# kocurvik/mdrp

Hardware: AMD Instinct MI355X
Metric: image-pairs/sec (2000 corrs, 10k RANSAC iters) (higher is better)
Workload: dtype f64

## Files before the change

### mdrp_amd/csrc/mdrp_capi.hip

```cpp
#include "../../include/mdrp.h"
#include "mdrp_kernels.h"
#include "mdrp_classic.h"
#ifdef MDRP_SPLIT_TU
#define MDRP_INST extern
#include "mdrp_instances.h"
namespace mdrp {
MDRP_INSTANCES_FINAL_64
MDRP_INSTANCES_FINAL_256
MDRP_INSTANCES_CLASSIC
}
#endif

#include <algorithm>
#include <cmath>
#include <cstdio>
#include <cstdlib>
#include <cstddef>
#include <cstring>
#include <functional>
#include <map>
#include <memory>
#include <mutex>
#include <string>
#include <vector>
// ... 342 lines not shown
    CamDev *d_cams1 = reinterpret_cast<CamDev *>(pd + sz.off_cam1), *d_cams2 = reinterpret_cast<CamDev *>(pd + sz.off_cam2);
    int32_t *d_table_n = reinterpret_cast<int32_t *>(pd + sz.off_tn), *d_table_of = reinterpret_cast<int32_t *>(pd + sz.off_tof),
            *d_nper = reinterpret_cast<int32_t *>(pd + sz.off_nper);
    Counters *cnt = h->counters.as<Counters>();
    const size_t groups_max = ((size_t)n_max + 15) / 16;
    const int trig_cap = chunk_cap;

    {
        unsigned char *ph = h->params_host;
        std::memcpy(ph, tab_state.data(), sizeof(uint64_t) * n_tables);
        const bool cams = kind == MDRP_CALIB || kind == MDRP_RELPOSE_5PT || kind == MDRP_SHARED_6PT;
        if (cams) { std::memcpy(ph + sz.off_cam1, cam1, sizeof(CamDev) * batch); std::memcpy(ph + sz.off_cam2, cam2 ? cam2 : cam1, sizeof(CamDev) * batch); }
        else std::memset(ph + sz.off_cam1, 0, 2 * sizeof(CamDev) * (size_t)batch);
        std::memcpy(ph + sz.off_tn, tab_n.data(), sizeof(int32_t) * n_tables);
        std::memcpy(ph + sz.off_tof, table_of.data(), sizeof(int32_t) * batch);
        std::memcpy(ph + sz.off_nper, n_host, sizeof(int32_t) * batch);
        HIPCHK(hipMemcpyAsync(pd, ph, sz.params, hipMemcpyHostToDevice, s));
    }
    HIPCHK(hipEventRecord(h->ev_tables, s));

    RunParams rp;
    std::memset(&rp, 0, sizeof rp);
    rp.kind = kind; rp.solver = solver_for(kind, est_shift); rp.est_shift = est_shift;
    rp.score_initial = ro->score_initial_model ? 1 : 0;
    rp.batch = batch; rp.n_max = n_max;
    rp.max_iterations = ro->max_iterations; rp.min_iterations = ro->min_iterations;
    rp.dyn_mult = ro->dyn_num_trials_mult; rp.log_prob_missing = std::log(1.0 - ro->success_prob);
    rp.weight_sampson = ro->monodepth_weight_sampson > 0.0f ? (double)ro->monodepth_weight_sampson : 0.0;
    rp.final_max_it = (int)std::min<uint64_t>(bo->max_iterations, 1u << 30); rp.final_loss = bo->loss_type;
    rp.grad_tol = bo->gradient_tol; rp.step_tol = bo->step_tol; rp.lambda0 = bo->initial_lambda;
    rp.lambda_min = bo->min_lambda; rp.lambda_max = bo->max_lambda;
    rp.chunk_len = chunk_cap; rp.chunk_off = 0; rp.slot_stride = chunk_cap * mps; rp.super_len = chunk_cap; rp.chunk_start = 0;
    rp.mps = mps; rp.sample_sz = ssz;

    auto launch_prep = [&](int p0, int pc, hipStream_t ps_) {
        const size_t o2 = (size_t)2 * p0 * n_max, o1 = (size_t)p0 * n_max;
        double *pts_p = h->pts.as<double>() + o1 * PT_STRIDE;
        uint4 *rfrag_p = h->rfrag.as<uint4>() + (size_t)p0 * groups_max * 64;
        if (classic)
            hipLaunchKernelGGL(kc_prep, dim3(pc), dim3(256), 0, ps_, rp, x1 + o2, x2 + o2, d_nper + p0, d_table_of + p0, d_cams1 + p0, d_cams2 + p0,
                               ro->max_epipolar_error, bo->loss_scale, pts_p, h->st.as<PairState>() + p0, rfrag_p);
        else
            hipLaunchKernelGGL(k_prep, dim3(pc), dim3(256), 0, ps_, rp, x1 + o2, x2 + o2, d1 + o1, d2 + o1, d_nper + p0, d_table_of + p0, d_cams1 + p0, d_cams2 + p0,
                               ro->max_epipolar_error, ro->max_reproj_error, bo->loss_scale, pts_p, h->dep.as<double>() + 2 * o1, h->st.as<PairState>() + p0, rfrag_p);
    };
    if (!host) {
        launch_prep(0, batch, s);
        HIPCHK(hipGetLastError());
    }
    rp.inl_stat = classic ? nullptr : &cnt->progress.wish_sum;

    const bool lo_overlap = env_int("MDRP_LO_OVERLAP", 1) != 0;
    const bool use_bound = env_int("MDRP_BOUND", 1) != 0;
    const int lo_threads = env_int("MDRP_LO_THREADS", (batch_call >= 128 && n_max < 4096) ? 64 : 256);
    const int final_threads = env_int("MDRP_FINAL_THREADS", batch_call >= 4096 ? 64 : 256);
    const int mask_index = lm_mask_index_on(n_max);
    const int clm_list_stride = lm_list_stride(n_max);
    const size_t clm_list_bytes = (size_t)2 * clm_list_stride * sizeof(uint16_t);
    const bool fuse_env = env_int("MDRP_FUSE_TAIL", ((kind == MDRP_CALIB && est_shift) || h->fuse_disabled) ? 0 : 1) != 0;
    bool final_done = false;
    auto launch_final = [&](const int32_t *ready, int32_t *fin_done, unsigned long long ticks, unsigned long long *timeouts) {
        if (classic)
            MDRP_CLASSIC_LM_DISPATCH(kc_final, final_threads, kind, dim3(batch), clm_list_bytes, s, rp, h->st.as<PairState>(), h->pts.as<double>(), mask_dev, results_dev,
                                     ready, fin_done, ticks, timeouts, clm_list_stride);
        else
            MDRP_FINAL_DISPATCH(final_threads, rp.final_loss, kind, est_shift, dim3(batch), (mask_index ? lm_final_list_bytes(n_max) : lm_list_bytes(n_max)), s, rp,
                                h->st.as<PairState>(), h->pts.as<double>(), h->dep.as<double>(), mask_dev, results_dev, lm_list_stride(n_max), mask_index,
                                h->lm_stats.as<unsigned long long>() + 2, ready, fin_done, ticks, timeouts);
    };
    const size_t tile_bytes = SCORE_TILE_BYTES;

    uint64_t it0 = 0;
    uint64_t max_needed = 0;
    while (true) {
        uint64_t lens[mdrp_handle::NC_MAX] = {0};
        int n_chunks = 1;
        if (it0 < certain) {
            const uint64_t span = std::min<uint64_t>(certain - it0, (uint64_t)chunk_cap);
            uint64_t used = 0;
            n_chunks = 0;
            if (it0 == 0)
                for (uint64_t l : lead) {
                    if (used + 2 * l > span) break;
                    lens[n_chunks++] = l; used += l;
                }
            lens[n_chunks++] = span - used;
        } else {
            lens[0] = std::min<uint64_t>(std::min<uint64_t>(std::max<uint64_t>(max_needed, 256), ro->max_iterations - it0), (uint64_t)chunk_cap);
        }
        uint64_t super_len = 0;
        for (int c = 0; c < n_chunks; ++c) super_len += lens[c];
        if (it0 == 0) h->first_chunk = (int64_t)lens[0];
        rp.chunk_start = it0; rp.super_len = (int)super_len;
        HIPCHK(hipMemsetAsync(h->counters.p, 0, sizeof(Counters), s));
        if (it0 == 0) HIPCHK(hipMemsetAsync(h->cand_stat.p, 0, sizeof(unsigned long long) * 2 * batch, s));
        const bool piped = n_chunks > 1 && lo_overlap;
        const bool fuse_tail = fuse_env && piped && it0 + super_len >= ro->max_iterations;
        int32_t *fz_ctl = nullptr, *fz_done = nullptr, *fz_fin = nullptr, *fz_ready = nullptr;
        if (fuse_tail) {
            if ((rc = h->fuse.ensure(sz.fuse))) return rc;
            fz_ctl = h->fuse.as<int32_t>(); fz_done = fz_ctl + 16; fz_fin = fz_done + batch; fz_ready = fz_fin + batch;
        }
        hipStream_t aux = piped ? h->aux_stream : s, aux2 = piped ? h->aux_stream2 : s;
        int offs[mdrp_handle::NC_MAX] = {0};
        for (int c = 1; c < n_chunks; ++c) offs[c] = offs[c - 1] + (int)lens[c - 1];
        const int samp_threads = env_int("MDRP_SAMPLE_THREADS", ssz == 3 ? SAMP_THREADS : (ssz == 5 ? 512 : 256));
// ... 75 lines not shown
            int32_t *surv1 = h->surv_count.as<int32_t>() + p0, *surv2 = h->surv2_count.as<int32_t>() + p0;
            hipEvent_t e0, e1;
            int rc_;
            if ((rc_ = get_events(h, &e0, &e1, 0))) return rc_;
            unsigned long long *cstats = &cnt->progress.evals;
            {
                hipEvent_t c0, c1;
                if ((rc_ = get_events(h, &c0, &c1, 1))) return rc_;
                const bool two_phase = !(it0 == 0 && c == 0);
                unsigned long long *cand_stat = h->cand_stat.as<unsigned long long>() + 2 * (size_t)p0;
                uint32_t *tags_u = tags_sc;
                int32_t *und_part = reinterpret_cast<int32_t *>(h->tags_sorted[!odd].as<uint32_t>() + so), *und_cnt = h->und_count.as<int32_t>() + 2 * (size_t)p0;
                const uint4 *rfrag_p = h->rfrag.as<uint4>() + (size_t)p0 * groups_max * 64;
                hipLaunchKernelGGL(k_count_plan, dim3(1), dim3(PLAN_THREADS), 0, s, pc, st_p, mcount_c, 2, CNT_WG_MODELS, h->cplan.as<int32_t>(),
                                   surv1, (const int32_t *)nullptr, two_phase ? und_cnt : (int32_t *)nullptr);
                const dim3 cgrid((unsigned)pc * (unsigned)((len * mps + CNT_WG_MODELS - 1) / CNT_WG_MODELS));
                HIPCHK(hipEventRecord(c0, s));
                MDRP_SWEEP_DISPATCH(k_count, kind, cgrid, dim3(CNT_THREADS), 0, s, r, st_p, rfrag_p, models_p,
                                    tags_c, mcount_c, h->cplan.as<int32_t>(), tags_v, surv1, cstats, (int32_t *)nullptr, (const int32_t *)nullptr,
                                    1, tags_u, und_part, und_cnt, (const int32_t *)nullptr, cand_stat);
                if (two_phase) {
                    hipLaunchKernelGGL(k_count_plan, dim3(1), dim3(PLAN_THREADS), 0, s, pc, st_p, und_cnt, 2, CNT_WG_MODELS, h->cplan.as<int32_t>(),
                                       (int32_t *)nullptr, (const int32_t *)nullptr, (int32_t *)nullptr);
                    MDRP_SWEEP_DISPATCH(k_count, kind, cgrid, dim3(CNT_THREADS), 0, s, r, st_p, rfrag_p, models_p,
                                        tags_u, und_cnt, h->cplan.as<int32_t>(), tags_v, surv1, cstats, (int32_t *)nullptr, (const int32_t *)nullptr,
                                        2, (uint32_t *)nullptr, (int32_t *)nullptr, (int32_t *)nullptr, und_part, cand_stat);
                    h->count_launches++;
                }
                HIPCHK(hipEventRecord(c1, s));
                h->count_launches++;
            }
            const uint32_t *surv_tags = tags_v;
            const int32_t *surv_cnt = surv1;
            if (use_bound && batch_call > 16 && !(it0 == 0 && c == 0)) {
                hipLaunchKernelGGL(k_count_plan, dim3(1), dim3(PLAN_THREADS), 0, s, pc, st_p, surv1, 1, BND_THREADS, h->cplan.as<int32_t>(), surv2, (const int32_t *)nullptr);
                const dim3 bgrid((unsigned)pc * (unsigned)((len * mps + BND_THREADS - 1) / BND_THREADS));
                unsigned long long *bstats = &cnt->progress.evals_bound;
                hipEvent_t b0, b1;
                if ((rc_ = get_events(h, &b0, &b1, 4))) return rc_;
                HIPCHK(hipEventRecord(b0, s));
                MDRP_SWEEP_DISPATCH(k_bound, kind, bgrid, dim3(BND_THREADS), 0, s, r, st_p, pts_p, models_p, tags_v, surv1, h->cplan.as<int32_t>(), tags_c, surv2, bstats);
                HIPCHK(hipEventRecord(b1, s));
                surv_tags = tags_c; surv_cnt = surv2;
            }
            int32_t *plan = h->plan.as<int32_t>(), *totals = plan + 2 * (size_t)batch + 2;
            if (batch_call <= SCORE_WAVE_MAX_PAIRS) {
                hipLaunchKernelGGL(k_count_plan, dim3(1), dim3(PLAN_THREADS), 0, s, pc, st_p, surv_cnt, 1, SCW_THREADS / 64, plan, (int32_t *)nullptr, (const int32_t *)nullptr, (int32_t *)nullptr);
                hipLaunchKernelGGL(k_sort_tags, dim3(pc), dim3(256), 0, s, r, st_p, mcount_c, surv_cnt, surv_tags, tags_sc);
                HIPCHK(hipEventRecord(e0, s));
                const long long ub = (long long)pc * ((len * mps + SCW_THREADS / 64 - 1) / (SCW_THREADS / 64));
                const dim3 grid((unsigned)std::min<long long>(ub, (long long)h->num_cu * 32));
                MDRP_SWEEP_DISPATCH(k_score_w, kind, grid, dim3(SCW_THREADS), 0, s, r, st_p, pts_p, models_p, tags_sc, mcount_c,
                                    h->slot_score.as<double>() + so, h->slot_inl.as<int32_t>() + so, plan);
            } else {
                hipLaunchKernelGGL(k_sort_tags, dim3(pc), dim3(256), 0, s, r, st_p, mcount_c, surv_cnt, surv_tags, tags_sc);
                hipLaunchKernelGGL(k_plan, dim3(1), dim3(PLAN_THREADS), 0, s, pc, mcount_c, plan, totals);
                HIPCHK(hipEventRecord(e0, s));
                const dim3 grid((unsigned)pc * (unsigned)((len * mps + SCORE_THREADS - 1) / SCORE_THREADS));
                MDRP_SWEEP_DISPATCH(k_score, kind, grid, dim3(SCORE_THREADS), tile_bytes, s, r, st_p, pts_p, models_p, tags_sc, mcount_c,
                                    h->slot_score.as<double>() + so, h->slot_inl.as<int32_t>() + so, plan, totals);
            }
            HIPCHK(hipEventRecord(e1, s));
            h->sweep_launches++;
            Trigger *trig_p = h->triggers.as<Trigger>() + (size_t)p0 * trig_cap;
            unsigned long long *scan_stats = &cnt->progress.evals_sweep;
#define MDRP_SCAN(M, I) hipLaunchKernelGGL((k_scan<M, I>), dim3(pc), dim3(64), 0, s, r, st_p, h->slot_score.as<double>() + so, h->slot_inl.as<int32_t>() + so, trig_p, trig_cap, mcount_c, scan_stats)
            if (mps == 16) MDRP_SCAN(16, 1);
            else if (mps == 12) MDRP_SCAN(12, 1);
            else if (len >= 1024) MDRP_SCAN(4, 4);
            else MDRP_SCAN(4, 1);
#undef MDRP_SCAN
            return MDRP_OK;
        };
        bool solved1 = false;
        int swept0 = 0;
        if (host && it0 == 0) {
            const bool sliced = piped && n_chunks >= 2 && batch >= 2 * HOST_SLICE_PAIRS;
            const int sl = sliced ? HOST_SLICE_PAIRS : batch;
            for (int p0 = 0; p0 < batch; p0 += sl) {
                const int pc = std::min(sl, batch - p0);
                const size_t o2 = (size_t)2 * p0 * n_max, o1 = (size_t)p0 * n_max, n2 = sizeof(double) * 2 * (size_t)pc * n_max, n1 = sizeof(double) * (size_t)pc * n_max;
                hipStream_t cs = sliced ? h->copy_stream : s;
                HIPCHK(hipMemcpyAsync(const_cast<double *>(x1) + o2, host->x1 + o2, n2, hipMemcpyHostToDevice, cs));
                HIPCHK(hipMemcpyAsync(const_cast<double *>(x2) + o2, host->x2 + o2, n2, hipMemcpyHostToDevice, cs));
                if (host->d1 && host->d2) {
                    HIPCHK(hipMemcpyAsync(const_cast<double *>(d1) + o1, host->d1 + o1, n1, hipMemcpyHostToDevice, cs));
                    HIPCHK(hipMemcpyAsync(const_cast<double *>(d2) + o1, host->d2 + o1, n1, hipMemcpyHostToDevice, cs));
                }
                if (!sliced) { launch_prep(p0, pc, s); break; }
                HIPCHK(hipEventRecord(h->ev_copied, cs)); HIPCHK(hipStreamWaitEvent(aux, h->ev_copied, 0));
                if (p0 == 0) HIPCHK(hipStreamWaitEvent(aux, h->ev_tables, 0));
                launch_prep(p0, pc, aux);
                HIPCHK(hipEventRecord(h->ev_prepped, aux));
                if ((rc = issue_solve(1, aux, p0, pc))) return rc;
                const bool last = p0 + sl >= batch, last_but_one = !last && p0 + 2 * sl >= batch;
                if (last_but_one || last) HIPCHK(hipStreamWaitEvent(s, h->ev_prepped, 0));
                auto solve_first = [&](int q0, int qc) -> int {
                    if (kind != MDRP_SHARED_6PT) return issue_solve(0, s, q0, qc);
                    int rc_ = issue_solve(0, aux, q0, qc);
                    if (rc_) return rc_;
                    HIPCHK(hipEventRecord(h->ev_solved6, aux));
                    HIPCHK(hipStreamWaitEvent(s, h->ev_solved6, 0));
                    return MDRP_OK;
                };
                if (last_but_one) { swept0 = p0 + pc; if ((rc = solve_first(0, swept0)) || (rc = sweep_chunk(0, 0, swept0))) return rc; }
                if (last) { if ((rc = solve_first(swept0, batch - swept0)) || (rc = sweep_chunk(0, swept0, batch - swept0))) return rc; swept0 = batch; }
            }
            if (sliced) { HIPCHK(hipEventRecord(h->ev_solved[1], aux)); solved1 = true; }
        }
// ... 430 lines not shown
        hipLaunchKernelGGL(kc_solver_unit<CLASSIC_SHARED>, dim3((count + 63) / 64), dim3(64), 0, s, count, h->unit_a.as<double>(),
                           h->unit_b.as<double>(), h->unit_e.as<Model>(), h->unit_f.as<int32_t>());
    else if (kind == MDRP_RELPOSE_5PT)
        hipLaunchKernelGGL(kc_solver_unit<CLASSIC_RELPOSE>, dim3((count + 63) / 64), dim3(64), SOLVE5_LDS_BYTES, s, count, h->unit_a.as<double>(),
                           h->unit_b.as<double>(), h->unit_e.as<Model>(), h->unit_f.as<int32_t>());
    else
        hipLaunchKernelGGL(kc_solver_unit<CLASSIC_FUND>, dim3((count + 63) / 64), dim3(64), SOLVE7_LDS_BYTES, s, count, h->unit_a.as<double>(),
                           h->unit_b.as<double>(), h->unit_e.as<Model>(), h->unit_f.as<int32_t>());
    HIPCHK(hipGetLastError());
    HIPCHK(hipMemcpyAsync(out, h->unit_e.p, sizeof(Model) * M * count, hipMemcpyDeviceToHost, s));
    HIPCHK(hipMemcpyAsync(n_out, h->unit_f.p, sizeof(int32_t) * count, hipMemcpyDeviceToHost, s));
    HIPCHK(hipStreamSynchronize(s));
    return MDRP_OK;
}

int mdrp_score_models(mdrp_handle *h, int kind, int mem_space, const mdrp_model *models, int num_models, const double *x1,
                      const double *x2, int n, double sq_threshold, double *scores, int32_t *counts) {
    if (!h || num_models < 0 || n < 0 || kind < 0 || kind > 5 || !scores || !counts) { g_err = "invalid argument"; return MDRP_ERR_INVALID; }
    if (num_models == 0) return MDRP_OK;
    MDRP_ENTER(h);
    hipStream_t s = h->stream;
    const int chunk = (num_models + 3) / 4;
    const size_t slots = (size_t)chunk * 4;
    int rc;
    if ((rc = h->pts.ensure(sizeof(double) * PT_STRIDE * std::max(n, 1))) || (rc = h->st.ensure(sizeof(PairState))) ||
        (rc = h->models.ensure(sizeof(Model) * slots)) || (rc = h->slot_score.ensure(sizeof(double) * slots)) ||
        (rc = h->slot_inl.ensure(sizeof(int32_t) * slots)) || (rc = h->tags[0].ensure(sizeof(uint32_t) * slots)) ||
        (rc = h->model_count[0].ensure(2 * sizeof(int32_t))))
        return rc;
    const double *x1d = x1, *x2d = x2;
    const Model *md = reinterpret_cast<const Model *>(models);
    if (mem_space == MDRP_MEM_HOST) {
        if ((rc = h->in_x1.ensure(sizeof(double) * 2 * std::max(n, 1))) || (rc = h->in_x2.ensure(sizeof(double) * 2 * std::max(n, 1)))) return rc;
        HIPCHK(hipMemcpyAsync(h->in_x1.p, x1, sizeof(double) * 2 * n, hipMemcpyHostToDevice, s));
        HIPCHK(hipMemcpyAsync(h->in_x2.p, x2, sizeof(double) * 2 * n, hipMemcpyHostToDevice, s));
        HIPCHK(hipMemcpyAsync(h->models.p, models, sizeof(Model) * num_models, hipMemcpyHostToDevice, s));
        x1d = h->in_x1.as<double>(); x2d = h->in_x2.as<double>();
        md = h->models.as<Model>();
    } else {
        HIPCHK(hipMemcpyAsync(h->models.p, models, sizeof(Model) * num_models, hipMemcpyDeviceToDevice, s));
        md = h->models.as<Model>();
    }
    if ((rc = upload_iota(s, h->tags[0].p, num_models))) return rc;
    const int32_t counts2[2] = {num_models, 0};
    HIPCHK(hipMemcpyAsync(h->model_count[0].p, counts2, 2 * sizeof(int32_t), hipMemcpyHostToDevice, s));
    if ((rc = stage_unit_pair(h, x1d, x2d, n, sq_threshold))) return rc;
    RunParams rp;
    std::memset(&rp, 0, sizeof rp);
    rp.kind = kind; rp.batch = 1; rp.n_max = std::max(n, 1); rp.chunk_len = chunk; rp.chunk_off = 0; rp.slot_stride = chunk * 4; rp.super_len = chunk;
    rp.mps = 4; rp.sample_sz = 3;
    const size_t tile_bytes = SCORE_TILE_BYTES;
    if ((rc = h->plan.ensure(sizeof(int32_t) * 8))) return rc;
    int32_t *plan = h->plan.as<int32_t>(), *totals = plan + 4;
    hipLaunchKernelGGL(k_plan, dim3(1), dim3(PLAN_THREADS), 0, s, 1, h->model_count[0].as<int32_t>(), plan, totals);
    const dim3 grid((unsigned)std::min(h->num_cu * 4, (num_models + SCORE_THREADS - 1) / SCORE_THREADS));
    h->ev_used = 0; h->sweep_launches = 1; h->sweep_evals = (int64_t)num_models * n;
    hipEvent_t e0, e1;
    if ((rc = get_events(h, &e0, &e1))) return rc;
    HIPCHK(hipEventRecord(e0, s));
    MDRP_SWEEP_DISPATCH(k_score, kind, grid, dim3(SCORE_THREADS), tile_bytes, s, rp, h->st.as<PairState>(), h->pts.as<double>(), md,
                        h->tags[0].as<uint32_t>(), h->model_count[0].as<int32_t>(), h->slot_score.as<double>(), h->slot_inl.as<int32_t>(), plan, totals);
    HIPCHK(hipEventRecord(e1, s));
    HIPCHK(hipGetLastError());
    const hipMemcpyKind back = mem_space == MDRP_MEM_HOST ? hipMemcpyDeviceToHost : hipMemcpyDeviceToDevice;
    HIPCHK(hipMemcpyAsync(scores, h->slot_score.p, sizeof(double) * num_models, back, s));
    HIPCHK(hipMemcpyAsync(counts, h->slot_inl.p, sizeof(int32_t) * num_models, back, s));
    return finish_timing(h);
}

int mdrp_count_candidates(mdrp_handle *h, int kind, const mdrp_model *models, int num_models, const double *x1, const double *x2,
                          int n, double sq_threshold, int32_t *candidates) {
    if (!h || num_models < 0 || n < 0 || kind < 0 || kind > 5 || !candidates || !models) { g_err = "invalid argument"; return MDRP_ERR_INVALID; }
    if (num_models == 0) return MDRP_OK;
    MDRP_ENTER(h);
    hipStream_t s = h->stream;
    const int nn = std::max(n, 1);
    const size_t slots = (size_t)num_models;
    int rc;
    if ((rc = h->pts.ensure(sizeof(double) * PT_STRIDE * nn)) || (rc = h->st.ensure(sizeof(PairState))) ||
        (rc = h->models.ensure(sizeof(Model) * slots)) || (rc = h->slot_inl.ensure(sizeof(int32_t) * slots)) ||
        (rc = h->tags[0].ensure(sizeof(uint32_t) * slots)) || (rc = h->tags_v.ensure(sizeof(uint32_t) * slots)) ||
        (rc = h->model_count[0].ensure(2 * sizeof(int32_t))) || (rc = h->surv_count.ensure(sizeof(int32_t))) ||
        (rc = h->cplan.ensure(2 * sizeof(int32_t))) || (rc = h->rfrag.ensure((size_t)((nn + 15) / 16) * 1024)) ||
        (rc = h->unit_f.ensure(sizeof(int32_t) * slots)) || (rc = h->in_x1.ensure(sizeof(double) * 2 * nn)) ||
        (rc = h->in_x2.ensure(sizeof(double) * 2 * nn)))
        return rc;
    HIPCHK(hipMemcpyAsync(h->in_x1.p, x1, sizeof(double) * 2 * n, hipMemcpyHostToDevice, s));
    HIPCHK(hipMemcpyAsync(h->in_x2.p, x2, sizeof(double) * 2 * n, hipMemcpyHostToDevice, s));
    HIPCHK(hipMemcpyAsync(h->models.p, models, sizeof(Model) * num_models, hipMemcpyHostToDevice, s));
    if ((rc = upload_iota(s, h->tags[0].p, num_models))) return rc;
    const int32_t counts2[2] = {num_models, 0};
    HIPCHK(hipMemcpyAsync(h->model_count[0].p, counts2, 2 * sizeof(int32_t), hipMemcpyHostToDevice, s));
    HIPCHK(hipMemsetAsync(h->surv_count.p, 0, sizeof(int32_t), s));
    if ((rc = stage_unit_pair(h, h->in_x1.as<double>(), h->in_x2.as<double>(), n, sq_threshold))) return rc;
    hipLaunchKernelGGL(k_frag_unit, dim3((n + 16 + 255) / 256), dim3(256), 0, s, n, h->pts.as<double>(), h->rfrag.as<uint4>());
    RunParams rp;
    std::memset(&rp, 0, sizeof rp);
    rp.kind = kind; rp.batch = 1; rp.n_max = nn; rp.slot_stride = num_models; rp.mps = 4; rp.sample_sz = 3;
    hipLaunchKernelGGL(k_count_plan, dim3(1), dim3(PLAN_THREADS), 0, s, 1, h->st.as<PairState>(), h->model_count[0].as<int32_t>(), 2, CNT_WG_MODELS, h->cplan.as<int32_t>(),
                       (int32_t *)nullptr);
    const dim3 grid((unsigned)((num_models + CNT_WG_MODELS - 1) / CNT_WG_MODELS));
    MDRP_SWEEP_DISPATCH(k_count, kind, grid, dim3(CNT_THREADS), 0, s, rp, h->st.as<PairState>(), h->rfrag.as<uint4>(), h->models.as<Model>(),
                        h->tags[0].as<uint32_t>(), h->model_count[0].as<int32_t>(), h->cplan.as<int32_t>(),
                        h->tags_v.as<uint32_t>(), h->surv_count.as<int32_t>(), (unsigned long long *)nullptr, h->unit_f.as<int32_t>());
    HIPCHK(hipGetLastError());
    HIPCHK(hipMemcpyAsync(candidates, h->unit_f.p, sizeof(int32_t) * num_models, hipMemcpyDeviceToHost, s));
    HIPCHK(hipStreamSynchronize(s));
// ... 95 lines not shown
```

### mdrp_amd/csrc/mdrp_kernels.h

```cpp
#pragma once
#include <hip/hip_runtime.h>
#include <float.h>
#include "mdrp_logtab.h"
#include "mdrp_math.h"

#ifdef MDRP_SECONDARY_TU
#define MDRP_GLOBAL static __global__
#else
#define MDRP_GLOBAL __global__
#endif

namespace mdrp {

constexpr int PT_STRIDE = 6;
#define MDRP_TILE_PTS 512
#define MDRP_SCORE_MINWAVES 4
constexpr int TILE_PTS = MDRP_TILE_PTS;
constexpr size_t SCORE_TILE_BYTES = (size_t)TILE_PTS * (PT_STRIDE * sizeof(double) + 4 * sizeof(float));
#define MDRP_P1F_UNROLL 8
#define MDRP_P1_UNROLL 4
constexpr int PRUNE_EVERY = 4;
#define MDRP_DENSE_KEY 40
#define MDRP_SOLVE_MINWAVES 2
#define MDRP_SCORE_THREADS 256
// ... 395 lines not shown
            const double *p = pts + idx * PT_STRIDE;
            s.x1[k][0] = p[0]; s.x1[k][1] = p[1]; s.x2[k][0] = p[2]; s.x2[k][1] = p[3];
            s.d1[k] = dep[2 * idx]; s.d2[k] = dep[2 * idx + 1];
        }
    };
    if (live) {
        Sample3 s;
        load_sample(s);
        n = run_solver(SOLVER, s, out);
    }
    if (SOLVER == SOLVER_P3P) {
        const unsigned long long valid = __ballot(live && n > 0);
        const int first_valid = valid ? __ffsll((long long)valid) - 1 : 64;
        if (live && (int)(threadIdx.x & 63) < first_valid) {
            Sample3 s;
            load_sample(s);
            nan_model = p3p_reference_nan(s);
        }
    }
    const int lane = threadIdx.x & 63;
    int pre = n;
#pragma unroll
    for (int o = 1; o < 64; o <<= 1) {
        const int v = __shfl_up(pre, o, 64);
        if (lane >= o) pre += v;
    }
    const int tot = __shfl(pre, 63, 64);
    int base = 0;
    if (lane == 63 && tot > 0) base = atomicAdd(&model_count[2 * pair], tot);
    base = __shfl(base, 63, 64);
    if (!live) return;
    const size_t slot0 = (size_t)pair * rp.slot_stride + (size_t)(rp.chunk_off + it) * 4;
    int pos = base + pre - n;
    const size_t tag_base = (size_t)pair * rp.slot_stride;
    *reinterpret_cast<int4 *>(slot_inl + slot0) = make_int4(nan_model ? -3 : (n > 0 ? -2 : -1), n > 1 ? -2 : -1, n > 2 ? -2 : -1, n > 3 ? -2 : -1);
    if (nan_model) {
        Model m;
        model_identity(m);
        const double qnan = __longlong_as_double(0x7ff8000000000000ll);
        m.q[0] = m.q[1] = m.q[2] = m.q[3] = m.t[0] = m.t[1] = m.t[2] = m.scale = qnan;
        models[slot0] = m;
    }
#pragma unroll
    for (int k = 0; k < 4; ++k) {
        if (k < n) {
            models[slot0 + k] = out[k];
            tags[tag_base + pos] = (uint32_t)((rp.chunk_off + it) * 4 + k);
            ++pos;
        }
    }
}

template <bool POSE>
__device__ __forceinline__ void score_point(const double *__restrict__ rec, const double E[9], const double R[9], const double t[3],
                                            double thr, double &score, int &cnt) {
    const double2 *P = reinterpret_cast<const double2 *>(rec);
    const double2 p01 = P[0], p23 = P[1];
    const double a = p01.x, b = p01.y, c = p23.x, d = p23.y;
    const SampsonTerms s = sampson_terms(E, a, b, c, d);
    if (!(s.C2 < thr * (1.0 + 1e-12) * s.den)) return;
    const double r2 = s.C2 / s.den;
    if (r2 < thr) {
        bool ok = true;
        if (POSE) {
            const double2 p45 = P[2];
            const double u0 = fma(R[0], a, fma(R[1], b, R[2]));
            const double u1 = fma(R[3], a, fma(R[4], b, R[5]));
            const double u2 = fma(R[6], a, fma(R[7], b, R[8]));
            const double uh = fma(u0, c, fma(u1, d, u2));
            const double ut = fma(u0, t[0], fma(u1, t[1], u2 * t[2]));
            const double ht = fma(c, t[0], fma(d, t[1], t[2]));
            const double A = -uh * p45.x * p45.y;
            const double b1 = -ut * p45.x, b2 = ht * p45.y;
            const double l1 = fma(-A, b2, b1), l2 = fma(-A, b1, b2);
            const double md = 0.01 * fma(-A, A, 1.0);
            ok = (l1 > md) && (l2 > md);
        }
        if (ok) { score += r2; ++cnt; }
    }
}

struct Prune {
    long long rec_cnt;
    double rec_score;
    int n;
    int processed;
    bool dead;
    bool wave_dead;
};

template <bool POSE>
__device__ __forceinline__ void score_tile_dense(const double *__restrict__ recs, int npts, const double E[9], const Model *__restrict__ mp,
                                                 double thr, double &score, int &cnt, Prune &pr) {
    const double thr_hi = thr * (1.0 + 1e-12);
    double R[9], t[3] = {0, 0, 0};
#pragma unroll
    for (int i = 0; i < 9; ++i) R[i] = 0;
    if (POSE) {
        double q[4];
        q[0] = mp->q[0]; q[1] = mp->q[1]; q[2] = mp->q[2]; q[3] = mp->q[3];
        t[0] = mp->t[0]; t[1] = mp->t[1]; t[2] = mp->t[2];
        quat_to_R(q, R);
    }
    for (int p0 = 0; p0 < npts; p0 += 32 * PRUNE_EVERY) {
        const int g = min(32 * PRUNE_EVERY, npts - p0);
        if (!pr.dead) {
#pragma unroll 2
            for (int j = 0; j < g; ++j) {
                const double2 *P = reinterpret_cast<const double2 *>(recs + (size_t)(p0 + j) * PT_STRIDE);
                const double2 p01 = P[0], p23 = P[1];
                const double a = p01.x, b = p01.y, c = p23.x, d = p23.y;
                const SampsonTerms s = sampson_terms(E, a, b, c, d);
                if (s.C2 < thr_hi * s.den) {
                    const double r2 = s.C2 / s.den;
                    if (r2 < thr) {
                        bool ok = true;
                        if (POSE) {
                            const double2 p45 = P[2];
                            const double u0 = fma(R[0], a, fma(R[1], b, R[2]));
                            const double u1 = fma(R[3], a, fma(R[4], b, R[5]));
                            const double u2 = fma(R[6], a, fma(R[7], b, R[8]));
                            const double uh = fma(u0, c, fma(u1, d, u2));
                            const double ut = fma(u0, t[0], fma(u1, t[1], u2 * t[2]));
                            const double ht = fma(c, t[0], fma(d, t[1], t[2]));
                            const double A = -uh * p45.x * p45.y;
                            const double b1 = -ut * p45.x, b2 = ht * p45.y;
                            const double l1 = fma(-A, b2, b1), l2 = fma(-A, b1, b2);
                            const double md = 0.01 * fma(-A, A, 1.0);
                            ok = (l1 > md) && (l2 > md);
                        }
                        if (ok) { score += r2; ++cnt; }
                    }
// ... 587 lines not shown
    const unsigned long long ball = __ballot(surv);
    if (ball) {
        int base = 0;
        const int first = __ffsll((long long)ball) - 1;
        if (lane == first) base = atomicAdd(&cnt_out[pair], __popcll(ball));
        base = __shfl(base, first, 64);
        if (surv) tags_out[slot_base + base + __popcll(ball & ((1ull << lane) - 1ull))] = tag;
    }
    if (stats && tid == 0 && blk == 0) atomicAdd(stats, (unsigned long long)cnt * (unsigned long long)n);
}

MDRP_GLOBAL __launch_bounds__(256) void k_sort_tags(RunParams rp, const PairState *__restrict__ st, int32_t *__restrict__ model_count,
                                                   const int32_t *__restrict__ surv_count,
                                                   const uint32_t *__restrict__ tags, uint32_t *__restrict__ tags_sorted) {
    const int pair = blockIdx.x, tid = threadIdx.x;
    const PairState &ps = st[pair];
    if (!ps.active) return;
    __shared__ int s_hist[PROBE_PTS + 1], s_pos[PROBE_PTS + 1];
    __shared__ int s_dense;
    if (tid <= PROBE_PTS) s_hist[tid] = 0;
    if (tid == 0) s_dense = 0;
    __syncthreads();
    const int cnt = surv_count[pair];
    const size_t slot_base = (size_t)pair * rp.slot_stride;
    const uint32_t *src = tags + slot_base;
    uint32_t *dst = tags_sorted + slot_base;
    const int dense_min = ps.n >= 8 ? MDRP_DENSE_KEY : PROBE_PTS + 1;
    for (int i = tid; i < cnt; i += 256) atomicAdd(&s_hist[min(src[i] >> 24, (uint32_t)PROBE_PTS)], 1);
    __syncthreads();
    if (tid < 64) {
        const int v = tid < dense_min ? s_hist[tid] : 0;
        int incl = v;
#pragma unroll
        for (int o = 1; o < 64; o <<= 1) {
            const int u = __shfl_up(incl, o, 64);
            if (tid >= o) incl += u;
        }
        s_pos[tid] = incl - v;
        if (tid == 63) s_pos[64] = incl;
    }
    __syncthreads();
    const int cap = rp.slot_stride;
    for (int i = tid; i < cnt; i += 256) {
        const uint32_t t = src[i];
        const int key = (int)min(t >> 24, (uint32_t)PROBE_PTS);
        if (key >= dense_min) dst[cap - 1 - atomicAdd(&s_dense, 1)] = t & 0xFFFFFFu;
        else dst[atomicAdd(&s_pos[key], 1)] = t & 0xFFFFFFu;
    }
    __syncthreads();
    if (tid == 0) { model_count[2 * pair] = cnt - s_dense; model_count[2 * pair + 1] = s_dense; }
}

MDRP_GLOBAL __launch_bounds__(PLAN_THREADS) void k_plan(int batch, const int32_t *__restrict__ model_count, int32_t *__restrict__ plan,
                                                       int32_t *__restrict__ totals ) {
    __shared__ int s_w[PLAN_THREADS / 64 + 1];
    int run_d = 0, run_s = 0;
    int32_t *pd = plan, *psp = plan + batch + 1;
    for (int p0 = 0; p0 < batch; p0 += PLAN_THREADS) {
        const int p = p0 + threadIdx.x;
        int bd = 0, bs = 0;
        if (p < batch) {
            bs = (model_count[2 * p] + SCORE_THREADS - 1) / SCORE_THREADS;
            bd = (model_count[2 * p + 1] + SCORE_THREADS - 1) / SCORE_THREADS;
        }
        int tot_d, tot_s;
        const int ed = plan_block_scan(bd, tot_d, s_w), es = plan_block_scan(bs, tot_s, s_w);
        if (p < batch) { pd[p] = run_d + run_s + ed + es; psp[p] = bs; }
        run_d += tot_d;
        run_s += tot_s;
    }
    if (threadIdx.x == 0) { pd[batch] = run_d + run_s; psp[batch] = 0; totals[0] = run_d; totals[1] = run_d + run_s; totals[2] = 0; }
}

template <bool POSE, bool RAWF = false>
__global__ __launch_bounds__(SCORE_THREADS, MDRP_SCORE_MINWAVES) void k_score(RunParams rp, const PairState *__restrict__ st, const double *__restrict__ pts,
                                                         const Model *__restrict__ models, const uint32_t *__restrict__ tags,
                                                         const int32_t *__restrict__ model_count, double *__restrict__ slot_score,
                                                         int32_t *__restrict__ slot_inl, const int32_t *__restrict__ plan,
                                                         int32_t *__restrict__ totals) {
    extern __shared__ double tile[];
    float4 *tile32 = reinterpret_cast<float4 *>(tile + TILE_PTS * PT_STRIDE);
    const int total = totals[1];
    const int tid = threadIdx.x;
    for (int w = blockIdx.x; w < total; w += gridDim.x) {
    const int pair = plan_find(plan, rp.batch, w);
    const int blk_sparse = plan[rp.batch + 1 + pair];
    const int bi = w - plan[pair];
    const bool dense = bi >= blk_sparse;
    const int blk = dense ? bi - blk_sparse : bi;
    const int cnt_sparse = model_count[2 * pair], cnt_dense = model_count[2 * pair + 1];
    const PairState &ps = st[pair];
    const int n = ps.n;
    const double thr = ps.sq_thr;
    const size_t slot_base = (size_t)pair * rp.slot_stride;
    const int cap = rp.slot_stride;
    bool live;
    uint32_t slot = 0;
    {
        const int i = blk * SCORE_THREADS + tid;
        live = i < (dense ? cnt_dense : cnt_sparse);
        if (live) slot = tags[slot_base + (dense ? cap - 1 - i : i)];
    }
    double E[9], thr_dmax;
    float tb, Ef[9];
    const Model *mp = models + slot_base + slot;
#pragma unroll
    for (int i = 0; i < 9; ++i) E[i] = 0;
    if (live) {
        const Model m = *mp;
        double R[9], Em[9];
        if (RAWF) {
#pragma unroll
            for (int i = 0; i < 9; ++i) E[i] = reinterpret_cast<const double *>(&m)[i];
        } else {
            quat_to_R(m.q, R);
            essential_from_Rt(R, m.t, Em);
// ... 55 lines not shown
        const int i = (w - plan[pair]) * (SCW_THREADS / 64) + wave;
        const int cnt_sparse = model_count[2 * pair], cnt_dense = model_count[2 * pair + 1];
        if (i >= cnt_sparse + cnt_dense) continue;
        const PairState &ps = st[pair];
        const int n = ps.n;
        const double thr = ps.sq_thr;
        const size_t slot_base = (size_t)pair * rp.slot_stride;
        const uint32_t slot = tags[slot_base + (i < cnt_sparse ? i : rp.slot_stride - 1 - (i - cnt_sparse))];
        const Model m = models[slot_base + slot];
        double E[9], R[9], t[3] = {m.t[0], m.t[1], m.t[2]};
#pragma unroll
        for (int q = 0; q < 9; ++q) R[q] = 0;
        if (RAWF) {
#pragma unroll
            for (int q = 0; q < 9; ++q) E[q] = reinterpret_cast<const double *>(&m)[q];
        } else {
            double Em[9];
            quat_to_R(m.q, R);
            essential_from_Rt(R, m.t, Em);
            if (POSE) {
#pragma unroll
                for (int q = 0; q < 9; ++q) E[q] = Em[q];
            } else fundamental_from_E(Em, m.f1, m.f2, E);
        }
        const long long rec_cnt = (long long)ps.best_min_cnt;
        const double rec_score = ps.best_min_score < DBL_MAX ? ps.best_min_score * (1.0 + 1e-12) : DBL_MAX;
        const double *gp = pts + (size_t)pair * rp.n_max * PT_STRIDE;
        double score = 0;
        int cnt = 0;
        bool pruned = false;
        for (int t0 = 0; t0 < n; t0 += 64) {
            const int r = t0 + lane;
            double s1 = 0;
            int c1 = 0;
            if (r < n) score_point<POSE>(gp + (size_t)r * PT_STRIDE, E, R, t, thr, s1, c1);
            const unsigned long long ball = __ballot(c1 != 0);
            if (ball) {
                if (c1) s_r2[wave][__popcll(ball & lt)] = s1;
                __builtin_amdgcn_fence(__ATOMIC_RELEASE, "wavefront");
                __builtin_amdgcn_wave_barrier();
                __builtin_amdgcn_fence(__ATOMIC_ACQUIRE, "wavefront");
                const int k = __popcll(ball);
                for (int j = 0; j < k; ++j) score += s_r2[wave][j];
                cnt += k;
                __builtin_amdgcn_wave_barrier();
            }
            const int processed = min(t0 + 64, n);
            if (rec_score < DBL_MAX && ((processed & 127) == 0 || processed == n) &&
                (long long)cnt + (long long)(n - processed) <= rec_cnt && score + thr * (double)(processed - cnt) >= rec_score) { pruned = true; break; }
        }
        if (lane == 0) {
            slot_score[slot_base + slot] = pruned ? DBL_MAX : score + thr * (double)(n - cnt);
            slot_inl[slot_base + slot] = pruned ? -2 : cnt;
        }
    }
}

template <int MPS = 4, int IPL = 1>
__global__ __launch_bounds__(64) void k_scan(RunParams rp, PairState *__restrict__ st, const double *__restrict__ slot_score,
                                             const int32_t *__restrict__ slot_inl, Trigger *__restrict__ triggers,
                                             int trig_cap, const int32_t *__restrict__ model_count,
                                             unsigned long long *__restrict__ evals) {
    const int pair = blockIdx.x, lane = threadIdx.x;
    PairState &ps = st[pair];
    if (!ps.active) { if (lane == 0) ps.n_triggers = 0; return; }
    if (lane == 0 && evals) atomicAdd(evals, (unsigned long long)(model_count[2 * pair] + model_count[2 * pair + 1]) * (unsigned long long)ps.n);
    long long run_cnt = (long long)ps.best_min_cnt;
    double run_score = ps.best_min_score;
    const double nan_score = (double)ps.n * ps.sq_thr;
    int ntrig = rp.chunk_off > 0 ? ps.n_triggers : 0;
    static_assert(MPS % 4 == 0, "slots of an iteration are read as 16-byte groups");
    constexpr int NG = MPS / 4;
    const size_t slot_base = (size_t)pair * rp.slot_stride + (size_t)rp.chunk_off * MPS;
    struct Slots { int4 c[IPL][NG]; double2 s01[IPL][NG], s23[IPL][NG]; };
    auto fetch = [&](int it0) {
        Slots r;
#pragma unroll
        for (int j = 0; j < IPL; ++j) {
            const int it = it0 + IPL * lane + j;
#pragma unroll
            for (int g = 0; g < NG; ++g) {
                if (it < rp.chunk_len) {
                    r.c[j][g] = *reinterpret_cast<const int4 *>(slot_inl + slot_base + (size_t)it * MPS + 4 * g);
                    const double2 *sp = reinterpret_cast<const double2 *>(slot_score + slot_base + (size_t)it * MPS + 4 * g);
                    r.s01[j][g] = sp[0]; r.s23[j][g] = sp[1];
                } else { r.c[j][g] = make_int4(-1, -1, -1, -1); r.s01[j][g] = r.s23[j][g] = make_double2(DBL_MAX, DBL_MAX); }
            }
        }
        return r;
    };
    Slots nxt = fetch(0);
    for (int it0 = 0; it0 < rp.chunk_len; it0 += 64 * IPL) {
        const Slots cur = nxt;
        if (it0 + 64 * IPL < rp.chunk_len) nxt = fetch(it0 + 64 * IPL);
        int c[IPL][MPS];
        double s[IPL][MPS];
        long long lc = -1;
        double ls = DBL_MAX;
#pragma unroll
        for (int j = 0; j < IPL; ++j) {
#pragma unroll
            for (int g = 0; g < NG; ++g) {
                c[j][4 * g] = cur.c[j][g].x; c[j][4 * g + 1] = cur.c[j][g].y; c[j][4 * g + 2] = cur.c[j][g].z; c[j][4 * g + 3] = cur.c[j][g].w;
                s[j][4 * g] = c[j][4 * g] >= 0 ? cur.s01[j][g].x : DBL_MAX; s[j][4 * g + 1] = c[j][4 * g + 1] >= 0 ? cur.s01[j][g].y : DBL_MAX;
                s[j][4 * g + 2] = c[j][4 * g + 2] >= 0 ? cur.s23[j][g].x : DBL_MAX; s[j][4 * g + 3] = c[j][4 * g + 3] >= 0 ? cur.s23[j][g].y : DBL_MAX;
            }
// ... 853 lines not shown
```

Measured before the change: 125,800.

## Add split-record scoring kernel sharing 64 hypotheses across four waves

Adds k_score_split, in which each 256-thread workgroup scores 64 hypotheses (one per lane) while its four waves split the correspondence records between them. Partial residuals are reduced through LDS, and wave 0 applies the early-bailout pruning and broadcasts a dead mask. Records are double-buffered in shared memory, and sparse hypotheses first pass an f32 prefilter. k_plan now takes the hypotheses-per-workgroup count as a parameter. The goal is better parallelism when each pair has few models, at the cost of extra __syncthreads and LDS traffic every step.

```diff
diff --git a/mdrp_amd/csrc/mdrp_capi.hip b/mdrp_amd/csrc/mdrp_capi.hip
--- a/mdrp_amd/csrc/mdrp_capi.hip
+++ b/mdrp_amd/csrc/mdrp_capi.hip
@@ -418,6 +418,7 @@
 
     const bool lo_overlap = env_int("MDRP_LO_OVERLAP", 1) != 0;
     const bool use_bound = env_int("MDRP_BOUND", 1) != 0;
+    const bool score_split = env_int("MDRP_SCORE_SPLIT", 1) != 0;
     const int lo_threads = env_int("MDRP_LO_THREADS", (batch_call >= 128 && n_max < 4096) ? 64 : 256);
     const int final_threads = env_int("MDRP_FINAL_THREADS", batch_call >= 4096 ? 64 : 256);
     const int mask_index = lm_mask_index_on(n_max);
@@ -599,9 +600,17 @@
                 const dim3 grid((unsigned)std::min<long long>(ub, (long long)h->num_cu * 32));
                 MDRP_SWEEP_DISPATCH(k_score_w, kind, grid, dim3(SCW_THREADS), 0, s, r, st_p, pts_p, models_p, tags_sc, mcount_c,
                                     h->slot_score.as<double>() + so, h->slot_inl.as<int32_t>() + so, plan);
+            } else if (score_split && !(it0 == 0 && c == 0)) {
+                hipLaunchKernelGGL(k_sort_tags, dim3(pc), dim3(256), 0, s, r, st_p, mcount_c, surv_cnt, surv_tags, tags_sc);
+                hipLaunchKernelGGL(k_plan, dim3(1), dim3(PLAN_THREADS), 0, s, pc, mcount_c, plan, totals, SPLIT_HYP);
+                HIPCHK(hipEventRecord(e0, s));
+                const long long ub = (long long)pc * ((len * mps + SPLIT_HYP - 1) / SPLIT_HYP + 1);
+                const dim3 grid((unsigned)std::min<long long>(ub, (long long)h->num_cu * 32));
+                MDRP_SWEEP_DISPATCH(k_score_split, kind, grid, dim3(SPLIT_THREADS), 0, s, r, st_p, pts_p, models_p, tags_sc, mcount_c,
+                                    h->slot_score.as<double>() + so, h->slot_inl.as<int32_t>() + so, plan, totals);
             } else {
                 hipLaunchKernelGGL(k_sort_tags, dim3(pc), dim3(256), 0, s, r, st_p, mcount_c, surv_cnt, surv_tags, tags_sc);
-                hipLaunchKernelGGL(k_plan, dim3(1), dim3(PLAN_THREADS), 0, s, pc, mcount_c, plan, totals);
+                hipLaunchKernelGGL(k_plan, dim3(1), dim3(PLAN_THREADS), 0, s, pc, mcount_c, plan, totals, SCORE_THREADS);
                 HIPCHK(hipEventRecord(e0, s));
                 const dim3 grid((unsigned)pc * (unsigned)((len * mps + SCORE_THREADS - 1) / SCORE_THREADS));
                 MDRP_SWEEP_DISPATCH(k_score, kind, grid, dim3(SCORE_THREADS), tile_bytes, s, r, st_p, pts_p, models_p, tags_sc, mcount_c,
@@ -1138,7 +1147,7 @@
     const size_t tile_bytes = SCORE_TILE_BYTES;
     if ((rc = h->plan.ensure(sizeof(int32_t) * 8))) return rc;
     int32_t *plan = h->plan.as<int32_t>(), *totals = plan + 4;
-    hipLaunchKernelGGL(k_plan, dim3(1), dim3(PLAN_THREADS), 0, s, 1, h->model_count[0].as<int32_t>(), plan, totals);
+    hipLaunchKernelGGL(k_plan, dim3(1), dim3(PLAN_THREADS), 0, s, 1, h->model_count[0].as<int32_t>(), plan, totals, SCORE_THREADS);
     const dim3 grid((unsigned)std::min(h->num_cu * 4, (num_models + SCORE_THREADS - 1) / SCORE_THREADS));
     h->ev_used = 0; h->sweep_launches = 1; h->sweep_evals = (int64_t)num_models * n;
     hipEvent_t e0, e1;
diff --git a/mdrp_amd/csrc/mdrp_kernels.h b/mdrp_amd/csrc/mdrp_kernels.h
--- a/mdrp_amd/csrc/mdrp_kernels.h
+++ b/mdrp_amd/csrc/mdrp_kernels.h
@@ -471,32 +471,37 @@
 }
 
 template <bool POSE>
-__device__ __forceinline__ void score_point(const double *__restrict__ rec, const double E[9], const double R[9], const double t[3],
-                                            double thr, double &score, int &cnt) {
+__device__ __forceinline__ bool record_inlier(const double *__restrict__ rec, const double E[9], const double R[9], const double t[3],
+                                              double thr, double &r2) {
     const double2 *P = reinterpret_cast<const double2 *>(rec);
     const double2 p01 = P[0], p23 = P[1];
     const double a = p01.x, b = p01.y, c = p23.x, d = p23.y;
     const SampsonTerms s = sampson_terms(E, a, b, c, d);
-    if (!(s.C2 < thr * (1.0 + 1e-12) * s.den)) return;
-    const double r2 = s.C2 / s.den;
-    if (r2 < thr) {
-        bool ok = true;
-        if (POSE) {
-            const double2 p45 = P[2];
-            const double u0 = fma(R[0], a, fma(R[1], b, R[2]));
-            const double u1 = fma(R[3], a, fma(R[4], b, R[5]));
-            const double u2 = fma(R[6], a, fma(R[7], b, R[8]));
-            const double uh = fma(u0, c, fma(u1, d, u2));
-            const double ut = fma(u0, t[0], fma(u1, t[1], u2 * t[2]));
-            const double ht = fma(c, t[0], fma(d, t[1], t[2]));
-            const double A = -uh * p45.x * p45.y;
-            const double b1 = -ut * p45.x, b2 = ht * p45.y;
-            const double l1 = fma(-A, b2, b1), l2 = fma(-A, b1, b2);
-            const double md = 0.01 * fma(-A, A, 1.0);
-            ok = (l1 > md) && (l2 > md);
-        }
-        if (ok) { score += r2; ++cnt; }
-    }
+    if (!(s.C2 < thr * (1.0 + 1e-12) * s.den)) return false;
+    r2 = s.C2 / s.den;
+    if (!(r2 < thr)) return false;
+    if (POSE) {
+        const double2 p45 = P[2];
+        const double u0 = fma(R[0], a, fma(R[1], b, R[2]));
+        const double u1 = fma(R[3], a, fma(R[4], b, R[5]));
+        const double u2 = fma(R[6], a, fma(R[7], b, R[8]));
+        const double uh = fma(u0, c, fma(u1, d, u2));
+        const double ut = fma(u0, t[0], fma(u1, t[1], u2 * t[2]));
+        const double ht = fma(c, t[0], fma(d, t[1], t[2]));
+        const double A = -uh * p45.x * p45.y;
+        const double b1 = -ut * p45.x, b2 = ht * p45.y;
+        const double l1 = fma(-A, b2, b1), l2 = fma(-A, b1, b2);
+        const double md = 0.01 * fma(-A, A, 1.0);
+        return (l1 > md) && (l2 > md);
+    }
+    return true;
+}
+
+template <bool POSE>
+__device__ __forceinline__ void score_point(const double *__restrict__ rec, const double E[9], const double R[9], const double t[3],
+                                            double thr, double &score, int &cnt) {
+    double r2;
+    if (record_inlier<POSE>(rec, E, R, t, thr, r2)) { score += r2; ++cnt; }
 }
 
 struct Prune {
@@ -1190,7 +1195,7 @@
 }
 
 MDRP_GLOBAL __launch_bounds__(PLAN_THREADS) void k_plan(int batch, const int32_t *__restrict__ model_count, int32_t *__restrict__ plan,
-                                                       int32_t *__restrict__ totals ) {
+                                                       int32_t *__restrict__ totals , int per_wg) {
     __shared__ int s_w[PLAN_THREADS / 64 + 1];
     int run_d = 0, run_s = 0;
     int32_t *pd = plan, *psp = plan + batch + 1;
@@ -1198,8 +1203,8 @@
         const int p = p0 + threadIdx.x;
         int bd = 0, bs = 0;
         if (p < batch) {
-            bs = (model_count[2 * p] + SCORE_THREADS - 1) / SCORE_THREADS;
-            bd = (model_count[2 * p + 1] + SCORE_THREADS - 1) / SCORE_THREADS;
+            bs = (model_count[2 * p] + per_wg - 1) / per_wg;
+            bd = (model_count[2 * p + 1] + per_wg - 1) / per_wg;
         }
         int tot_d, tot_s;
         const int ed = plan_block_scan(bd, tot_d, s_w), es = plan_block_scan(bs, tot_s, s_w);
@@ -1361,6 +1366,169 @@
         if (lane == 0) {
             slot_score[slot_base + slot] = pruned ? DBL_MAX : score + thr * (double)(n - cnt);
             slot_inl[slot_base + slot] = pruned ? -2 : cnt;
+        }
+    }
+}
+
+constexpr int SPLIT_THREADS = 256;
+constexpr int SPLIT_WAVES = SPLIT_THREADS / 64;
+constexpr int SPLIT_HYP = 64;
+constexpr int SPLIT_Q = 8;
+constexpr int SPLIT_STEP = SPLIT_WAVES * SPLIT_Q;
+static_assert(128 % SPLIT_STEP == 0, "the bail-out positions (every 128 records) must be step boundaries");
+template <bool POSE, bool RAWF = false>
+__global__ __launch_bounds__(SPLIT_THREADS, MDRP_SCORE_MINWAVES) void k_score_split(RunParams rp, const PairState *__restrict__ st, const double *__restrict__ pts,
+                                                               const Model *__restrict__ models, const uint32_t *__restrict__ tags ,
+                                                               const int32_t *__restrict__ model_count, double *__restrict__ slot_score,
+                                                               int32_t *__restrict__ slot_inl, const int32_t *__restrict__ plan ,
+                                                               const int32_t *__restrict__ totals) {
+    __shared__ double s_rec[2][SPLIT_WAVES][SPLIT_Q * PT_STRIDE];
+    __shared__ float4 s_rec32[2][SPLIT_WAVES][SPLIT_Q];
+    __shared__ double s_r2[2][SPLIT_STEP][SPLIT_HYP];
+    __shared__ int32_t s_cnt[2][SPLIT_WAVES][SPLIT_HYP];
+    __shared__ unsigned long long s_dead[2];
+    const int total = totals[1];
+    const int lane = threadIdx.x & 63;
+    const int wave = __builtin_amdgcn_readfirstlane(threadIdx.x >> 6);
+    for (int w = blockIdx.x; w < total; w += gridDim.x) {
+        const int pair = plan_find(plan, rp.batch, w);
+        const int blk_sparse = plan[rp.batch + 1 + pair];
+        const int bi = w - plan[pair];
+        const bool dense = bi >= blk_sparse;
+        const int blk = dense ? bi - blk_sparse : bi;
+        const int cnt_sparse = model_count[2 * pair], cnt_dense = model_count[2 * pair + 1];
+        const PairState &ps = st[pair];
+        const int n = ps.n;
+        const double thr = ps.sq_thr;
+        const size_t slot_base = (size_t)pair * rp.slot_stride;
+        const int i = blk * SPLIT_HYP + lane;
+        const bool live = i < (dense ? cnt_dense : cnt_sparse);
+        uint32_t slot = 0;
+        if (live) slot = tags[slot_base + (dense ? rp.slot_stride - 1 - i : i)];
+        double E[9], R[9], t[3] = {0, 0, 0};
+#pragma unroll
+        for (int q = 0; q < 9; ++q) { E[q] = 0; R[q] = 0; }
+        if (live) {
+            const Model m = models[slot_base + slot];
+            if (RAWF) {
+#pragma unroll
+                for (int q = 0; q < 9; ++q) E[q] = reinterpret_cast<const double *>(&m)[q];
+            } else {
+                double Em[9];
+                quat_to_R(m.q, R);
+                essential_from_Rt(R, m.t, Em);
+                t[0] = m.t[0]; t[1] = m.t[1]; t[2] = m.t[2];
+                if (POSE) {
+#pragma unroll
+                    for (int q = 0; q < 9; ++q) E[q] = Em[q];
+                } else fundamental_from_E(Em, m.f1, m.f2, E);
+            }
+        }
+        double thr_dmax;
+        float Ef[9], tb;
+        bound_setup(E, ps, thr, Ef, tb, thr_dmax);
+        const long long rec_cnt = (long long)ps.best_min_cnt;
+        const double rec_score = ps.best_min_score < DBL_MAX ? ps.best_min_score * (1.0 + 1e-12) : DBL_MAX;
+        const double *gp = pts + (size_t)pair * rp.n_max * PT_STRIDE;
+        const int steps = (n + SPLIT_STEP - 1) / SPLIT_STEP;
+        double2 nx = {0, 0};
+        auto fetch = [&](int j) {
+            const int r = j * SPLIT_STEP + wave * SPLIT_Q + lane / 3;
+            if (lane < 3 * SPLIT_Q && r < n) nx = reinterpret_cast<const double2 *>(gp + (size_t)r * PT_STRIDE)[lane % 3];
+        };
+        auto stage = [&](int j) {
+            const int k = lane / 3, part = lane % 3;
+            if (lane < 3 * SPLIT_Q && j * SPLIT_STEP + wave * SPLIT_Q + k < n) {
+                reinterpret_cast<double2 *>(s_rec[j & 1][wave])[lane] = nx;
+                float *q = reinterpret_cast<float *>(s_rec32[j & 1][wave]) + (k >> 1) * 8 + (k & 1);
+                if (part == 0) { q[0] = (float)nx.x; q[2] = (float)nx.y; }
+                else if (part == 1) { q[4] = (float)nx.x; q[6] = (float)nx.y; }
+            }
+        };
+        fetch(0);
+        stage(0);
+        __syncthreads();
+        double score = 0;
+        int cnt = 0;
+        bool dead = !live;
+        bool skip = !live;
+        for (int j = 0; j <= steps; ++j) {
+            if (j > 0) {
+                const unsigned long long dm = s_dead[(j - 1) & 1];
+                if (dm == ~0ull) break;
+                skip = (dm >> lane) & 1;
+            }
+            if (wave == 0) {
+                if (j > 0) {
+                    const int b = (j - 1) & 1;
+                    if (!dead) {
+#pragma unroll 1
+                        for (int q = 0; q < SPLIT_WAVES; ++q) {
+#pragma unroll
+                            for (int r = 0; r < SPLIT_Q; ++r) score += s_r2[b][q * SPLIT_Q + r][lane];
+                            cnt += s_cnt[b][q][lane];
+                        }
+                    }
+                    const int processed = min(j * SPLIT_STEP, n);
+                    if (rec_score < DBL_MAX && ((processed & 127) == 0 || processed == n))
+                        dead = dead || (((long long)cnt + (long long)(n - processed) <= rec_cnt) &&
+                                        (score + thr * (double)(processed - cnt) >= rec_score));
+                }
+                if (j < steps) {
+                    const unsigned long long dm = __ballot(dead);
+                    if (lane == 0) s_dead[j & 1] = dm;
+                }
+                skip = dead;
+            }
+            if (j == steps) break;
+            if (j + 1 < steps) fetch(j + 1);
+            const int b = j & 1;
+            const int valid = min(SPLIT_Q, n - (j * SPLIT_STEP + wave * SPLIT_Q));
+            const double *rec = s_rec[b][wave];
+            double *out = &s_r2[b][wave * SPLIT_Q][lane];
+            int found = 0;
+            if (dense) {
+#pragma unroll 2
+                for (int jj = 0; jj < SPLIT_Q; ++jj) {
+                    double v = 0.0, r2;
+                    if (jj < valid && !skip && record_inlier<POSE>(rec + jj * PT_STRIDE, E, R, t, thr, r2)) { v = r2; ++found; }
+                    out[jj * SPLIT_HYP] = v;
+                }
+            } else {
+#pragma unroll
+                for (int jj = 0; jj < SPLIT_Q; ++jj) out[jj * SPLIT_HYP] = 0.0;
+                const float4 *b32 = s_rec32[b][wave];
+                f32x2 Ev[9];
+#pragma unroll
+                for (int q = 0; q < 9; ++q) Ev[q] = (f32x2)(Ef[q]);
+                uint32_t mask = 0;
+#pragma unroll
+                for (int jj = 0; jj < SPLIT_Q; jj += 2) {
+                    const float4 ab = b32[jj], cd = b32[jj + 1];
+                    const f32x2 a = {ab.x, ab.y}, bb = {ab.z, ab.w}, c = {cd.x, cd.y}, d = {cd.z, cd.w};
+                    const f32x2 e0 = __builtin_elementwise_fma(Ev[0], a, __builtin_elementwise_fma(Ev[1], bb, Ev[2]));
+                    const f32x2 e1 = __builtin_elementwise_fma(Ev[3], a, __builtin_elementwise_fma(Ev[4], bb, Ev[5]));
+                    const f32x2 e2 = __builtin_elementwise_fma(Ev[6], a, __builtin_elementwise_fma(Ev[7], bb, Ev[8]));
+                    const f32x2 C = __builtin_elementwise_fma(c, e0, __builtin_elementwise_fma(d, e1, e2));
+                    mask |= (!(fabsf(C.x) > tb) ? 1u : 0u) << jj;
+                    mask |= (!(fabsf(C.y) > tb) ? 1u : 0u) << (jj + 1);
+                }
+                mask &= valid >= SPLIT_Q ? 0xFFu : (valid > 0 ? (1u << valid) - 1u : 0u);
+                if (skip) mask = 0;
+                while (mask) {
+                    const int jj = __ffs(mask) - 1;
+                    mask &= mask - 1;
+                    double r2;
+                    if (record_inlier<POSE>(rec + jj * PT_STRIDE, E, R, t, thr, r2)) { out[jj * SPLIT_HYP] = r2; ++found; }
+                }
+            }
+            s_cnt[b][wave][lane] = found;
+            if (j + 1 < steps) stage(j + 1);
+            __syncthreads();
+        }
+        if (wave == 0 && live) {
+            slot_score[slot_base + slot] = dead ? DBL_MAX : score + thr * (double)(n - cnt);
+            slot_inl[slot_base + slot] = dead ? -2 : cnt;
         }
     }
 }
```

New measurement: 130,800 (median of 6 runs). 1.04x the previous value.
